# Lainshower/debiasing-multi-modal

Measured on AMD Instinct MI355X. Metric: images/sec (embed+adapter step), CLIP-RN50 224px bs=1024, higher is better.
Workload: dtype f32; 1 GPU; CLIP-RN50 224px encode_image + adapter(1024-128-1024) CE/SGD step, 1024 images/GPU, global batch 1024 (the metric's configuration, CLIP-RN50 224px bs=1024 on one GPU); global_batch=1024, batch_per_gpu=1024, parallelism=dp1, collective=none

## Files before the change

debiasing-multi-modal_amd/csrc/conv_patch.hip:

```cpp
#include <stdlib.h>
#include "common.h"

namespace {

constexpr int TR = 4, TC = 28;
constexpr int PR = TR + 2, PC = TC + 2, PPX = PR * PC;
constexpr int CIN = 32, KTOT = 9 * CIN;
constexpr int WROW = KTOT + 8;

struct PatchP {
    const float* x; const float* x_absmax;
    const u16* w; int w_exp; const float* sc; const float* bias;
    float* y; float* y_absmax;
    int B, H, W, tiles_w, tiles_h, n_tiles;
};

__device__ __forceinline__ int pswz(int row) { return (row >> 2) & 3; }

template <int N, int POOL>
__global__ __launch_bounds__(256, N == 32 ? 3 : 2) void conv3x3_c32_kernel(const PatchP p) {
    constexpr int TN = N / 32, NLD = (PPX * 8 + 255) / 256;
    constexpr int PCL = POOL ? 40 : PC, PLN = PR * PCL * 32;
    __shared__ __attribute__((aligned(16))) u16 lds[N * WROW + 2 * PLN];
    u16* Wl = lds;
    u16* Pl = lds + N * WROW;
    const int tid = threadIdx.x, lane = tid & 63, wave = tid >> 6;
    const int fr = lane & 31, fh = lane >> 5;

    for (int i = tid; i < N * (KTOT / 8); i += 256) {
        const int n = i / (KTOT / 8), c = i - n * (KTOT / 8);
        *(u32x4*)(Wl + n * WROW + c * 8) = *(const u32x4*)(p.w + (size_t)n * KTOT + c * 8);
    }
    const int s_a = scale_exp(*p.x_absmax);
    const float a_sc = pow2f(s_a), acc_scale = pow2f(-s_a - p.w_exp);
    float sv[TN], bv[TN];
#pragma unroll
    for (int j = 0; j < TN; ++j) { sv[j] = p.sc[j * 32 + fr] * acc_scale; bv[j] = p.bias[j * 32 + fr]; }

    const int ml = wave * 32 + fr;
    int a_dy, a_c;
    bool a_ok;
    if (POOL) { const int o = ml >> 2, q = ml & 3; a_dy = 2 * (o / 14) + (q >> 1); a_c = 2 * (o % 14) + (q & 1); a_ok = ml < TR * TC; }
    else { a_dy = wave; a_c = fr; a_ok = fr < TC; }
    const int a_row0 = a_ok ? a_dy * PCL + a_c : 0;

    const long long img_bytes = (long long)p.H * p.W * CIN * 4;
    f32x4 pre[NLD];
    auto tile_coords = [&](int tile, int& b, int& h0, int& w0) {
        const int tw = tile % p.tiles_w, r = tile / p.tiles_w;
        b = r / p.tiles_h; h0 = (r - b * p.tiles_h) * TR; w0 = tw * TC;
    };
    auto load_patch = [&](int tile) {
        int b, h0, w0;
        tile_coords(tile, b, h0, w0);
        const __amdgpu_buffer_rsrc_t rs = desc(p.x, (long long)p.B * img_bytes, (long long)b * img_bytes);
#pragma unroll
        for (int k = 0; k < NLD; ++k) {
            const int idx = tid + 256 * k, i = idx >> 3, quad = idx & 7;
            const int py = i / PC, px = i - py * PC, h = h0 - 1 + py, w = w0 - 1 + px;
            const bool ok = i < PPX && h >= 0 && h < p.H && w >= 0 && w < p.W;
            pre[k] = __builtin_bit_cast(f32x4, __builtin_amdgcn_raw_buffer_load_b128(
                rs, ok ? (unsigned)((h * p.W + w) * (CIN * 4) + quad * 16) : OOR, 0, 0));
        }
    };
    auto store_patch = [&]() {
#pragma unroll
        for (int k = 0; k < NLD; ++k) {
            const int idx = tid + 256 * k, i = idx >> 3, quad = idx & 7;
            if (i < PPX) {
                unsigned hp[2], lp[2];
#pragma unroll
                for (int j = 0; j < 2; ++j) split2h_pair(pre[k][2 * j], pre[k][2 * j + 1], a_sc, hp[j], lp[j]);
                const int py = i / PC, row = py * PCL + (i - py * PC);
                const int off = row * 32 + (((quad >> 1) ^ pswz(row)) << 3) + ((quad & 1) << 2);
                *(u32x2*)(Pl + off) = (u32x2){hp[0], hp[1]};
                *(u32x2*)(Pl + PLN + off) = (u32x2){lp[0], lp[1]};
            }
        }
    };

    float amax = 0.f;
    int tile = blockIdx.x;
    if (tile < p.n_tiles) load_patch(tile);
    for (; tile < p.n_tiles; tile += gridDim.x) {
        store_patch();
        __syncthreads();
        if (tile + (int)gridDim.x < p.n_tiles) load_patch(tile + gridDim.x);

        f32x16 acc[TN];
#pragma unroll
        for (int j = 0; j < TN; ++j)
#pragma unroll
            for (int r = 0; r < 16; ++r) acc[j][r] = 0.f;
#pragma unroll
        for (int tap = 0; tap < 9; ++tap) {
            const int row = a_row0 + (tap / 3) * PCL + (tap % 3);
#pragma unroll
            for (int ks = 0; ks < 2; ++ks) {
                const int aoff = row * 32 + (((2 * ks + fh) ^ pswz(row)) << 3);
                const u32x4 ah = *(const u32x4*)(Pl + aoff), al = *(const u32x4*)(Pl + PLN + aoff);
                u32x4 wf[TN];
#pragma unroll
                for (int j = 0; j < TN; ++j) wf[j] = *(const u32x4*)(Wl + (j * 32 + fr) * WROW + tap * 32 + (2 * ks + fh) * 8);
#pragma unroll
                for (int j = 0; j < TN; ++j)
                    acc[j] = __builtin_amdgcn_mfma_f32_32x32x16_f16(__builtin_bit_cast(f16x8, al), __builtin_bit_cast(f16x8, wf[j]), acc[j], 0, 0, 0);
#pragma unroll
                for (int j = 0; j < TN; ++j)
                    acc[j] = __builtin_amdgcn_mfma_f32_32x32x16_f16(__builtin_bit_cast(f16x8, ah), __builtin_bit_cast(f16x8, wf[j]), acc[j], 0, 0, 0);
            }
        }
        int b, h0, w0;
        tile_coords(tile, b, h0, w0);
        if constexpr (POOL) {
            const int Hp = p.H >> 1, Wp = p.W >> 1;
            const long long tot = (long long)p.B * Hp * Wp * N * 4;
            const long long base_px = ((long long)b * Hp + (h0 >> 1)) * Wp + (w0 >> 1);
            const __amdgpu_buffer_rsrc_t rs = desc(p.y, tot, base_px * N * 4);
#pragma unroll
            for (int t = 0; t < 4; ++t) {
                const int o = wave * 8 + 2 * t + fh;
                const unsigned off = o < 28 ? (unsigned)(((o / 14) * Wp + (o % 14)) * (N * 4) + fr * 4) : OOR;
#pragma unroll
                for (int j = 0; j < TN; ++j) {
                    float v[4];
#pragma unroll
                    for (int q = 0; q < 4; ++q) v[q] = fmaxf(fmaf(acc[j][4 * t + q], sv[j], bv[j]), 0.f);
                    const float s = (((v[0] + v[1]) + v[2]) + v[3]) * 0.25f;
                    __builtin_amdgcn_raw_buffer_store_b32(__builtin_bit_cast(unsigned, s), rs, off, (unsigned)(j * 128), 0);
                    if (o < 28) amax = fmaxf(amax, fmaxf(fmaxf(v[0], v[1]), fmaxf(v[2], v[3])));
                }
            }
        } else {
            const long long tot = (long long)p.B * p.H * p.W * N * 4;
            const long long base_px = ((long long)b * p.H + h0) * p.W + w0;
            const __amdgpu_buffer_rsrc_t rs = desc(p.y, tot, base_px * N * 4);
#pragma unroll
            for (int r = 0; r < 16; ++r) {
                const int c = (r & 3) + 8 * (r >> 2) + 4 * fh, dy = wave;
                const bool m_ok = c < TC;
                const unsigned off = m_ok ? (unsigned)((dy * p.W + c) * (N * 4) + fr * 4) : OOR;
#pragma unroll
                for (int j = 0; j < TN; ++j) {
                    const float v = fmaxf(fmaf(acc[j][r], sv[j], bv[j]), 0.f);
                    __builtin_amdgcn_raw_buffer_store_b32(__builtin_bit_cast(unsigned, v), rs, off, (unsigned)(j * 128), 0);
                    if (m_ok) amax = fmaxf(amax, v);
                }
            }
        }
        __syncthreads();
    }
    if (p.y_absmax) {
        amax = wave_max(amax);
        float* red = (float*)Pl;
        if (lane == 0) red[wave] = amax;
        __syncthreads();
        if (tid == 0) {
            const float m = fmaxf(fmaxf(red[0], red[1]), fmaxf(red[2], red[3]));
            if (m > *(volatile const float*)p.y_absmax) atomicMax((unsigned*)p.y_absmax, __float_as_uint(m));
        }
    }
}

}

extern "C" int dbmm_conv3x3_c32_bn_relu_x2(const float* x, const float* x_absmax, const void* w_plane_f16, int w_exp,
                                           const float* scale, const float* bias, float* y, float* y_absmax, int64_t B, int64_t H,
                                           int64_t W, int64_t Cin, int64_t Cout, int pool, void* stream) {
    if (!x || !x_absmax || !w_plane_f16 || !scale || !bias || !y) return DBMM_E_ARG;
    if (B <= 0 || H <= 0 || W <= 0 || (pool != 0 && pool != 2)) return DBMM_E_SHAPE;
    if (Cin != CIN || (Cout != 32 && Cout != 64) || (H % TR) || (W % TC) || w_exp < -40 || w_exp > 40) return DBMM_E_UNSUPPORTED;
    if (H * W * CIN * 4 >= EXT_LIM || B * (H / TR) * (W / TC) > INT32_MAX) return DBMM_E_UNSUPPORTED;
    if (!dbmm_aligned16(x) || !dbmm_aligned16(w_plane_f16) || !dbmm_aligned16(y)) return DBMM_E_ALIGN;
    PatchP p{};
    p.x = x; p.x_absmax = x_absmax; p.w = (const u16*)w_plane_f16; p.w_exp = w_exp; p.sc = scale; p.bias = bias;
    p.y = y; p.y_absmax = y_absmax; p.B = (int)B; p.H = (int)H; p.W = (int)W;
    p.tiles_w = (int)(W / TC); p.tiles_h = (int)(H / TR); p.n_tiles = (int)(B * p.tiles_h * p.tiles_w);
    const int per_cu = Cout == 32 ? 3 : 2;
    const int grid = p.n_tiles < DBMM_N_CU * per_cu ? p.n_tiles : DBMM_N_CU * per_cu;
    hipStream_t s = (hipStream_t)stream;
    if (Cout == 32) {
        if (pool) hipLaunchKernelGGL((conv3x3_c32_kernel<32, 1>), dim3(grid), dim3(256), 0, s, p);
        else hipLaunchKernelGGL((conv3x3_c32_kernel<32, 0>), dim3(grid), dim3(256), 0, s, p);
    } else {
        if (pool) hipLaunchKernelGGL((conv3x3_c32_kernel<64, 1>), dim3(grid), dim3(256), 0, s, p);
        else hipLaunchKernelGGL((conv3x3_c32_kernel<64, 0>), dim3(grid), dim3(256), 0, s, p);
    }
    DBMM_CHECK_LAUNCH();
    return DBMM_OK;
}
```

debiasing-multi-modal_amd/csrc/options.hip:

```cpp
#include <atomic>
#include <ctype.h>
#include <stdlib.h>
#include <string.h>
#include "common.h"

namespace {

struct OptDef { const char* name; int def; };
const OptDef kOpts[DBMM_OPT_COUNT] = {
    {"igemm_epi_direct", 1},
    {"igemm_fast", 1},
    {"igemm_streamk", 1},
    {"igemm_x3", 1},
    {"igemm_x2", 1},
    {"igemm_x2_bk", 32},
    {"igemm_bk", 0},
    {"igemm_halo", 1},
    {"igemm_halo_pool", 2},
    {"igemm_bn256", 1},
    {"igemm_bn256_kxk", 1},
    {"gemm_8ph", 1},
    {"f16_8ph", 1},
    {"f16_bn256", 1},
    {"stem_mfma", 1},
    {"mha_valu", 0},
    {"conv_patch", 1},
    {"mha_x2", 1},
    {"adapter_step_fused", 1},
    {"conv1x1_stream", 1},
    {"conv1x1_8ph", 1},
    {"chain8", 0},
    {"conv1x1_bn256", 0},
    {"tail_split", 1},
    {"halo8", 1},
    {"dual_8ph", 1},
    {"mha_short", 1},
    {"f16_conv_8ph", 1},
    {"conv1x1_res_stream", 1},
    {"linear_step_one_launch_max_b", 512},
};

std::atomic<int> g_val[DBMM_OPT_COUNT];

struct Seed {
    Seed() {
        for (int i = 0; i < DBMM_OPT_COUNT; ++i) {
            char env[64] = "DBMM_";
            size_t n = strlen(env);
            for (const char* c = kOpts[i].name; *c && n + 1 < sizeof(env); ++c) env[n++] = (char)toupper((unsigned char)*c);
            env[n] = 0;
            const char* e = getenv(env);
            g_val[i].store(e ? atoi(e) : kOpts[i].def, std::memory_order_relaxed);
        }
    }
} g_seed;

int find(const char* name) {
    if (!name) return -1;
    for (int i = 0; i < DBMM_OPT_COUNT; ++i)
        if (!strcmp(name, kOpts[i].name)) return i;
    return -1;
}

}

int dbmm_opt(int id) { return g_val[id].load(std::memory_order_relaxed); }

extern "C" int dbmm_set_option(const char* name, int value) {
    const int i = find(name);
    if (i < 0) return DBMM_E_ARG;
    g_val[i].store(value, std::memory_order_relaxed);
    return DBMM_OK;
}

extern "C" int dbmm_get_option(const char* name, int* value) {
    const int i = find(name);
    if (i < 0 || !value) return DBMM_E_ARG;
    *value = g_val[i].load(std::memory_order_relaxed);
    return DBMM_OK;
}
```

Before: 37090 images/sec.

## Add software-pipelined 3x3 patch conv with register-resident weights for pooled Cout=64

After: 37150 images/sec (median of 6 runs). About the same (+0.2%).

```diff
diff --git a/debiasing-multi-modal_amd/csrc/conv_patch.hip b/debiasing-multi-modal_amd/csrc/conv_patch.hip
--- a/debiasing-multi-modal_amd/csrc/conv_patch.hip
+++ b/debiasing-multi-modal_amd/csrc/conv_patch.hip
@@ -7,6 +7,7 @@
 constexpr int PR = TR + 2, PC = TC + 2, PPX = PR * PC;
 constexpr int CIN = 32, KTOT = 9 * CIN;
 constexpr int WROW = KTOT + 8;
+constexpr int WROW_H = KTOT / 2 + 8;
 
 struct PatchP {
     const float* x; const float* x_absmax;
@@ -17,13 +18,89 @@
 
 __device__ __forceinline__ int pswz(int row) { return (row >> 2) & 3; }
 
+#ifdef PATCH_STAMP
+__device__ long long g_patch_stamps[16];
+__device__ long long g_patch_span[2 * 1024];
+#define SPAN_START const long long span_t0 = wall_clock64()
+#define STAMP_DECL const bool stamp_on = blockIdx.x == 8 && threadIdx.x < 64; long long st[8] = {0, 0, 0, 0, 0, 0, 0, 0}, tprev = clock64(), ntl = 0
+#define STAMP(i) do { if (stamp_on) { const long long now__ = clock64(); st[i] += now__ - tprev; tprev = now__; } } while (0)
+#define STAMP_VMCNT(n) asm volatile("s_waitcnt vmcnt(%0)" :: "n"(n) : "memory")
+#define STAMP_LGKM0() asm volatile("s_waitcnt lgkmcnt(0)" ::: "memory")
+#define STAMP_TILE() (++ntl)
+#define STAMP_END() do { if (stamp_on && threadIdx.x == 0) { for (int i = 0; i < 8; ++i) g_patch_stamps[i] = st[i]; g_patch_stamps[8] = ntl; } \
+                         if (threadIdx.x == 0 && blockIdx.x < 1024) { g_patch_span[2 * blockIdx.x] = span_t0; g_patch_span[2 * blockIdx.x + 1] = wall_clock64(); } } while (0)
+#else
+#define SPAN_START do { } while (0)
+#define STAMP_DECL do { } while (0)
+#define STAMP(i) do { } while (0)
+#define STAMP_VMCNT(n) do { } while (0)
+#define STAMP_LGKM0() do { } while (0)
+#define STAMP_TILE() do { } while (0)
+#define STAMP_END() do { } while (0)
+#endif
+
 template <int N, int POOL>
-__global__ __launch_bounds__(256, N == 32 ? 3 : 2) void conv3x3_c32_kernel(const PatchP p) {
+__device__ __forceinline__ void patch_epilogue(const PatchP& p, const f32x16 (&acc)[N / 32], const float (&sv)[N / 32], const float (&bv)[N / 32],
+                                               int b, int h0, int w0, int wave, int fr, int fh, float& amax) {
+    constexpr int TN = N / 32;
+    if constexpr (POOL) {
+        const int Hp = p.H >> 1, Wp = p.W >> 1;
+        const long long tot = (long long)p.B * Hp * Wp * N * 4;
+        const long long base_px = ((long long)b * Hp + (h0 >> 1)) * Wp + (w0 >> 1);
+        const __amdgpu_buffer_rsrc_t rs = desc(p.y, tot, base_px * N * 4);
+#pragma unroll
+        for (int t = 0; t < 4; ++t) {
+            const int o = wave * 8 + 2 * t + fh;
+            const unsigned off = o < 28 ? (unsigned)(((o / 14) * Wp + (o % 14)) * (N * 4) + fr * 4) : OOR;
+#pragma unroll
+            for (int j = 0; j < TN; ++j) {
+                float v[4];
+#pragma unroll
+                for (int q = 0; q < 4; ++q) v[q] = fmaxf(fmaf(acc[j][4 * t + q], sv[j], bv[j]), 0.f);
+                const float s = (((v[0] + v[1]) + v[2]) + v[3]) * 0.25f;
+                __builtin_amdgcn_raw_buffer_store_b32(__builtin_bit_cast(unsigned, s), rs, off, (unsigned)(j * 128), 0);
+                if (o < 28) amax = fmaxf(amax, fmaxf(fmaxf(v[0], v[1]), fmaxf(v[2], v[3])));
+            }
+        }
+    } else {
+        const long long tot = (long long)p.B * p.H * p.W * N * 4;
+        const long long base_px = ((long long)b * p.H + h0) * p.W + w0;
+        const __amdgpu_buffer_rsrc_t rs = desc(p.y, tot, base_px * N * 4);
+#pragma unroll
+        for (int r = 0; r < 16; ++r) {
+            const int c = (r & 3) + 8 * (r >> 2) + 4 * fh, dy = wave;
+            const bool m_ok = c < TC;
+            const unsigned off = m_ok ? (unsigned)((dy * p.W + c) * (N * 4) + fr * 4) : OOR;
+#pragma unroll
+            for (int j = 0; j < TN; ++j) {
+                const float v = fmaxf(fmaf(acc[j][r], sv[j], bv[j]), 0.f);
+                __builtin_amdgcn_raw_buffer_store_b32(__builtin_bit_cast(unsigned, v), rs, off, (unsigned)(j * 128), 0);
+                if (m_ok) amax = fmaxf(amax, v);
+            }
+        }
+    }
+}
+
+__device__ __forceinline__ void patch_absmax_out(const PatchP& p, float amax, float* red, int tid) {
+    if (p.y_absmax) {
+        amax = wave_max(amax);
+        if ((tid & 63) == 0) red[tid >> 6] = amax;
+        __syncthreads();
+        if (tid == 0) {
+            const float m = fmaxf(fmaxf(red[0], red[1]), fmaxf(red[2], red[3]));
+            if (m > *(volatile const float*)p.y_absmax) atomicMax((unsigned*)p.y_absmax, __float_as_uint(m));
+        }
+    }
+}
+
+template <int N, int POOL>
+__global__ __launch_bounds__(256, N == 32 ? 3 : 2) void conv3x3_c32_kernel_v1(const PatchP p) {
     constexpr int TN = N / 32, NLD = (PPX * 8 + 255) / 256;
     constexpr int PCL = POOL ? 40 : PC, PLN = PR * PCL * 32;
     __shared__ __attribute__((aligned(16))) u16 lds[N * WROW + 2 * PLN];
     u16* Wl = lds;
     u16* Pl = lds + N * WROW;
+    SPAN_START;
     const int tid = threadIdx.x, lane = tid & 63, wave = tid >> 6;
     const int fr = lane & 31, fh = lane >> 5;
 
@@ -82,10 +159,17 @@
     float amax = 0.f;
     int tile = blockIdx.x;
     if (tile < p.n_tiles) load_patch(tile);
+    STAMP_DECL;
     for (; tile < p.n_tiles; tile += gridDim.x) {
+        STAMP_VMCNT(TN * (POOL ? 4 : 16));
+        STAMP(0);
         store_patch();
+        STAMP_LGKM0();
+        STAMP(1);
         __syncthreads();
+        STAMP(2);
         if (tile + (int)gridDim.x < p.n_tiles) load_patch(tile + gridDim.x);
+        STAMP(3);
 
         f32x16 acc[TN];
 #pragma unroll
@@ -110,59 +194,175 @@
                     acc[j] = __builtin_amdgcn_mfma_f32_32x32x16_f16(__builtin_bit_cast(f16x8, ah), __builtin_bit_cast(f16x8, wf[j]), acc[j], 0, 0, 0);
             }
         }
+        STAMP(4);
         int b, h0, w0;
         tile_coords(tile, b, h0, w0);
-        if constexpr (POOL) {
-            const int Hp = p.H >> 1, Wp = p.W >> 1;
-            const long long tot = (long long)p.B * Hp * Wp * N * 4;
-            const long long base_px = ((long long)b * Hp + (h0 >> 1)) * Wp + (w0 >> 1);
-            const __amdgpu_buffer_rsrc_t rs = desc(p.y, tot, base_px * N * 4);
-#pragma unroll
-            for (int t = 0; t < 4; ++t) {
-                const int o = wave * 8 + 2 * t + fh;
-                const unsigned off = o < 28 ? (unsigned)(((o / 14) * Wp + (o % 14)) * (N * 4) + fr * 4) : OOR;
-#pragma unroll
-                for (int j = 0; j < TN; ++j) {
-                    float v[4];
-#pragma unroll
-                    for (int q = 0; q < 4; ++q) v[q] = fmaxf(fmaf(acc[j][4 * t + q], sv[j], bv[j]), 0.f);
-                    const float s = (((v[0] + v[1]) + v[2]) + v[3]) * 0.25f;
-                    __builtin_amdgcn_raw_buffer_store_b32(__builtin_bit_cast(unsigned, s), rs, off, (unsigned)(j * 128), 0);
-                    if (o < 28) amax = fmaxf(amax, fmaxf(fmaxf(v[0], v[1]), fmaxf(v[2], v[3])));
-                }
-            }
-        } else {
-            const long long tot = (long long)p.B * p.H * p.W * N * 4;
-            const long long base_px = ((long long)b * p.H + h0) * p.W + w0;
-            const __amdgpu_buffer_rsrc_t rs = desc(p.y, tot, base_px * N * 4);
-#pragma unroll
-            for (int r = 0; r < 16; ++r) {
-                const int c = (r & 3) + 8 * (r >> 2) + 4 * fh, dy = wave;
-                const bool m_ok = c < TC;
-                const unsigned off = m_ok ? (unsigned)((dy * p.W + c) * (N * 4) + fr * 4) : OOR;
-#pragma unroll
-                for (int j = 0; j < TN; ++j) {
-                    const float v = fmaxf(fmaf(acc[j][r], sv[j], bv[j]), 0.f);
-                    __builtin_amdgcn_raw_buffer_store_b32(__builtin_bit_cast(unsigned, v), rs, off, (unsigned)(j * 128), 0);
-                    if (m_ok) amax = fmaxf(amax, v);
-                }
-            }
-        }
+        patch_epilogue<N, POOL>(p, acc, sv, bv, b, h0, w0, wave, fr, fh, amax);
+        STAMP(5);
         __syncthreads();
-    }
-    if (p.y_absmax) {
-        amax = wave_max(amax);
-        float* red = (float*)Pl;
-        if (lane == 0) red[wave] = amax;
+        STAMP(6);
+        STAMP_TILE();
+    }
+    STAMP_END();
+    patch_absmax_out(p, amax, (float*)Pl, tid);
+}
+
+template <int N, int POOL>
+__global__ __launch_bounds__(256, 2) void conv3x3_c32_kernel(const PatchP p) {
+    static_assert(N == 64, "k-step-0 fragments of two column blocks in registers");
+    constexpr int TN = N / 32, NLD = (PPX * 8 + 255) / 256;
+    constexpr int PF = 1;
+    constexpr int WP = WROW_H;
+    constexpr int PCL = POOL ? 40 : PC, PLN = PR * PCL * 32, PBUF = 2 * PLN;
+    static_assert(NLD <= 8, "one patch chunk per tap, taps 1 .. NLD");
+    __shared__ __attribute__((aligned(16))) u16 lds[N * WP + 2 * PBUF];
+    u16* Wl = lds;
+    u16* Pl = lds + N * WP;
+    SPAN_START;
+    const int tid = threadIdx.x, lane = tid & 63, wave = tid >> 6;
+    const int fr = lane & 31, fh = lane >> 5;
+
+    u32x4 wr[9][TN];
+    for (int i = tid; i < N * 18; i += 256) {
+        const int n = i / 18, c = i - n * 18;
+        *(u32x4*)(Wl + n * WP + c * 8) = *(const u32x4*)(p.w + (size_t)n * KTOT + (c >> 1) * 32 + 16 + (c & 1) * 8);
+    }
+#pragma unroll
+    for (int tap = 0; tap < 9; ++tap)
+#pragma unroll
+        for (int j = 0; j < TN; ++j) wr[tap][j] = *(const u32x4*)(p.w + (size_t)(j * 32 + fr) * KTOT + tap * 32 + fh * 8);
+    const int s_a = scale_exp(*p.x_absmax);
+    const float a_sc = pow2f(s_a), acc_scale = pow2f(-s_a - p.w_exp);
+    float sv[TN], bv[TN];
+#pragma unroll
+    for (int j = 0; j < TN; ++j) { sv[j] = p.sc[j * 32 + fr] * acc_scale; bv[j] = p.bias[j * 32 + fr]; }
+
+    const int ml = wave * 32 + fr;
+    int a_dy, a_c;
+    bool a_ok;
+    if (POOL) { const int o = ml >> 2, q = ml & 3; a_dy = 2 * (o / 14) + (q >> 1); a_c = 2 * (o % 14) + (q & 1); a_ok = ml < TR * TC; }
+    else { a_dy = wave; a_c = fr; a_ok = fr < TC; }
+    const int a_row0 = a_ok ? a_dy * PCL + a_c : 0;
+
+    const long long img_bytes = (long long)p.H * p.W * CIN * 4;
+    int tile = blockIdx.x;
+    const int t_end = p.n_tiles, G = (int)gridDim.x;
+    f32x4 pre[NLD];
+    auto tile_coords = [&](int tile, int& b, int& h0, int& w0) {
+        const int tw = tile % p.tiles_w, r = tile / p.tiles_w;
+        b = r / p.tiles_h; h0 = (r - b * p.tiles_h) * TR; w0 = tw * TC;
+    };
+    auto load_chunk = [&](int k, const __amdgpu_buffer_rsrc_t rs, int h0, int w0, bool live) {
+        const int idx = tid + 256 * k, i = idx >> 3, quad = idx & 7;
+        const int py = i / PC, px = i - py * PC, h = h0 - 1 + py, w = w0 - 1 + px;
+        const bool ok = live & (i < PPX) & ((unsigned)h < (unsigned)p.H) & ((unsigned)w < (unsigned)p.W);
+        pre[k] = __builtin_bit_cast(f32x4, __builtin_amdgcn_raw_buffer_load_b128(
+            rs, (unsigned)((h * p.W + w) * (CIN * 4) + quad * 16) | (ok ? 0u : OOR), 0, 0));
+    };
+    auto store_chunk = [&](int k, u16* Pd) {
+        const int idx = tid + 256 * k, i = idx >> 3, quad = idx & 7;
+        if (255 + 256 * k < PPX * 8 || i < PPX) {
+            unsigned hp[2], lp[2];
+#pragma unroll
+            for (int j = 0; j < 2; ++j) split2h_pair(pre[k][2 * j], pre[k][2 * j + 1], a_sc, hp[j], lp[j]);
+            const int py = i / PC, row = py * PCL + (i - py * PC);
+            const int off = row * 32 + (((quad >> 1) ^ pswz(row)) << 3) + ((quad & 1) << 2);
+            *(u32x2*)(Pd + off) = (u32x2){hp[0], hp[1]};
+            *(u32x2*)(Pd + PLN + off) = (u32x2){lp[0], lp[1]};
+        }
+    };
+
+    float amax = 0.f;
+    {
+        int b, h0, w0;
+        tile_coords(tile, b, h0, w0);
+        const __amdgpu_buffer_rsrc_t rs = desc(p.x, (long long)p.B * img_bytes, (long long)b * img_bytes);
+#pragma unroll
+        for (int k = 0; k < NLD; ++k) load_chunk(k, rs, h0, w0, tile < t_end);
+#pragma unroll
+        for (int k = 0; k < NLD; ++k) store_chunk(k, Pl);
+        const bool live = t_end - tile > G;
+        tile_coords(live ? tile + G : tile, b, h0, w0);
+        const __amdgpu_buffer_rsrc_t rs1 = desc(p.x, (long long)p.B * img_bytes, (long long)b * img_bytes);
+#pragma unroll
+        for (int k = 0; k < NLD; ++k) load_chunk(k, rs1, h0, w0, live);
+    }
+    int cur = 0;
+    __syncthreads();
+    STAMP_DECL;
+    for (; tile < t_end; tile += G) {
+        const u16* Pc = Pl + cur;
+        u16* Pn = Pl + (PBUF - cur);
+        const bool live2 = t_end - tile > 2 * G;
+        int b2, h2, w2;
+        tile_coords(live2 ? tile + 2 * G : tile, b2, h2, w2);
+        const __amdgpu_buffer_rsrc_t rs2 = desc(p.x, (long long)p.B * img_bytes, (long long)b2 * img_bytes);
+
+        f32x16 acc[TN];
+#pragma unroll
+        for (int j = 0; j < TN; ++j)
+#pragma unroll
+            for (int r = 0; r < 16; ++r) acc[j][r] = 0.f;
+        u32x4 fa[PF + 1][2], fw[PF + 1][TN];
+        auto read_frags = [&](int s) {
+            const int tap = s >> 1, ks = s & 1;
+            const int row = a_row0 + (tap / 3) * PCL + (tap % 3);
+            const int aoff = row * 32 + (((2 * ks + fh) ^ pswz(row)) << 3);
+            fa[s % (PF + 1)][0] = *(const u32x4*)(Pc + aoff); fa[s % (PF + 1)][1] = *(const u32x4*)(Pc + PLN + aoff);
+#pragma unroll
+            for (int j = 0; j < TN; ++j) {
+                if (ks) fw[s % (PF + 1)][j] = *(const u32x4*)(Wl + (j * 32 + fr) * WP + tap * 16 + fh * 8);
+            }
+        };
+#pragma unroll
+        for (int s = 0; s < PF; ++s) read_frags(s);
+#pragma unroll
+        for (int s = 0; s < 18; ++s) {
+            const int tap = s >> 1, ks = s & 1;
+            if (s + PF < 18) read_frags(s + PF);
+            __builtin_amdgcn_sched_barrier(0);
+            const u32x4 ah = fa[s % (PF + 1)][0], al = fa[s % (PF + 1)][1];
+            u32x4 wf[TN];
+#pragma unroll
+            for (int j = 0; j < TN; ++j) wf[j] = ks ? fw[s % (PF + 1)][j] : wr[tap][j];
+#pragma unroll
+            for (int j = 0; j < TN; ++j)
+                acc[j] = __builtin_amdgcn_mfma_f32_32x32x16_f16(__builtin_bit_cast(f16x8, al), __builtin_bit_cast(f16x8, wf[j]), acc[j], 0, 0, 0);
+            if (tap >= 1 && tap <= NLD) {
+                if (!ks) store_chunk(tap - 1, Pn);
+                else load_chunk(tap - 1, rs2, h2, w2, live2);
+            }
+#pragma unroll
+            for (int j = 0; j < TN; ++j)
+                acc[j] = __builtin_amdgcn_mfma_f32_32x32x16_f16(__builtin_bit_cast(f16x8, ah), __builtin_bit_cast(f16x8, wf[j]), acc[j], 0, 0, 0);
+            __builtin_amdgcn_sched_barrier(0);
+        }
+        STAMP(4);
+        int b, h0, w0;
+        tile_coords(tile, b, h0, w0);
+        patch_epilogue<N, POOL>(p, acc, sv, bv, b, h0, w0, wave, fr, fh, amax);
+        STAMP(5);
+        cur = PBUF - cur;
         __syncthreads();
-        if (tid == 0) {
-            const float m = fmaxf(fmaxf(red[0], red[1]), fmaxf(red[2], red[3]));
-            if (m > *(volatile const float*)p.y_absmax) atomicMax((unsigned*)p.y_absmax, __float_as_uint(m));
-        }
-    }
-}
-
-}
+        STAMP(6);
+        STAMP_TILE();
+    }
+    STAMP_END();
+    patch_absmax_out(p, amax, (float*)Pl, tid);
+}
+
+}
+
+#ifdef PATCH_STAMP
+extern "C" void dbmm_debug_patch_stamps(long long* out ) {
+    (void)hipDeviceSynchronize();
+    (void)hipMemcpyFromSymbol(out, HIP_SYMBOL(g_patch_stamps), 16 * sizeof(long long));
+}
+extern "C" void dbmm_debug_patch_spans(long long* out ) {
+    (void)hipDeviceSynchronize();
+    (void)hipMemcpyFromSymbol(out, HIP_SYMBOL(g_patch_span), 2 * 1024 * sizeof(long long));
+}
+#endif
 
 extern "C" int dbmm_conv3x3_c32_bn_relu_x2(const float* x, const float* x_absmax, const void* w_plane_f16, int w_exp,
                                            const float* scale, const float* bias, float* y, float* y_absmax, int64_t B, int64_t H,
@@ -176,15 +376,21 @@
     p.x = x; p.x_absmax = x_absmax; p.w = (const u16*)w_plane_f16; p.w_exp = w_exp; p.sc = scale; p.bias = bias;
     p.y = y; p.y_absmax = y_absmax; p.B = (int)B; p.H = (int)H; p.W = (int)W;
     p.tiles_w = (int)(W / TC); p.tiles_h = (int)(H / TR); p.n_tiles = (int)(B * p.tiles_h * p.tiles_w);
+    hipStream_t s = (hipStream_t)stream;
+    if (dbmm_opt(OPT_CONV_PATCH) >= 2 && Cout == 64 && pool) {
+        const int grid = p.n_tiles < DBMM_N_CU * 2 ? p.n_tiles : DBMM_N_CU * 2;
+        hipLaunchKernelGGL((conv3x3_c32_kernel<64, 1>), dim3(grid), dim3(256), 0, s, p);
+        DBMM_CHECK_LAUNCH();
+        return DBMM_OK;
+    }
     const int per_cu = Cout == 32 ? 3 : 2;
     const int grid = p.n_tiles < DBMM_N_CU * per_cu ? p.n_tiles : DBMM_N_CU * per_cu;
-    hipStream_t s = (hipStream_t)stream;
     if (Cout == 32) {
-        if (pool) hipLaunchKernelGGL((conv3x3_c32_kernel<32, 1>), dim3(grid), dim3(256), 0, s, p);
-        else hipLaunchKernelGGL((conv3x3_c32_kernel<32, 0>), dim3(grid), dim3(256), 0, s, p);
+        if (pool) hipLaunchKernelGGL((conv3x3_c32_kernel_v1<32, 1>), dim3(grid), dim3(256), 0, s, p);
+        else hipLaunchKernelGGL((conv3x3_c32_kernel_v1<32, 0>), dim3(grid), dim3(256), 0, s, p);
     } else {
-        if (pool) hipLaunchKernelGGL((conv3x3_c32_kernel<64, 1>), dim3(grid), dim3(256), 0, s, p);
-        else hipLaunchKernelGGL((conv3x3_c32_kernel<64, 0>), dim3(grid), dim3(256), 0, s, p);
+        if (pool) hipLaunchKernelGGL((conv3x3_c32_kernel_v1<64, 1>), dim3(grid), dim3(256), 0, s, p);
+        else hipLaunchKernelGGL((conv3x3_c32_kernel_v1<64, 0>), dim3(grid), dim3(256), 0, s, p);
     }
     DBMM_CHECK_LAUNCH();
     return DBMM_OK;
diff --git a/debiasing-multi-modal_amd/csrc/options.hip b/debiasing-multi-modal_amd/csrc/options.hip
--- a/debiasing-multi-modal_amd/csrc/options.hip
+++ b/debiasing-multi-modal_amd/csrc/options.hip
@@ -24,7 +24,7 @@
     {"f16_bn256", 1},
     {"stem_mfma", 1},
     {"mha_valu", 0},
-    {"conv_patch", 1},
+    {"conv_patch", 2},
     {"mha_x2", 1},
     {"adapter_step_fused", 1},
     {"conv1x1_stream", 1},
```
